# dsmyl6/OpenPyStruct

Measured on AMD Instinct MI355X. Metric: beam FE solves/s (100-elem, batched), higher is better.
Workload: dtype f64

## Files before the change

openpystruct_amd/build.py:

```python
from __future__ import annotations

import os
import shutil
import subprocess
import sys

PKG = os.path.dirname(os.path.abspath(__file__))
ROOT = os.path.dirname(PKG)
CSRC = os.path.join(PKG, "csrc")
LIB = os.path.join(PKG, "lib", "libopenpystruct_amd.so")
SOURCES = [os.path.join(CSRC, "beam_solve.hip"), os.path.join(CSRC, "beam_fat.hip"), os.path.join(CSRC, "sizing_step.hip"),
           os.path.join(CSRC, "beam_residual.hip"), os.path.join(CSRC, "frame_solve.hip"),
           os.path.join(CSRC, "stencil_bn.hip"), os.path.join(CSRC, "flat_adam.hip"),
           os.path.join(CSRC, "fused_loss.hip"), os.path.join(CSRC, "fused_bn.hip"), os.path.join(CSRC, "input_prep.hip"),
           os.path.join(CSRC, "mlp_block.hip"), os.path.join(CSRC, "seq_block.hip"), os.path.join(CSRC, "seq_layer.hip"), os.path.join(CSRC, "mem_bench.hip"), os.path.join(CSRC, "case_draw.hip"),
           os.path.join(CSRC, "bayes_mlp.hip"), os.path.join(CSRC, "beam_vjp.hip"), os.path.join(CSRC, "frame_vjp.hip"), os.path.join(CSRC, "sizing_grad.hip"),
           os.path.join(CSRC, "frame_sizing_grad.hip"), os.path.join(CSRC, "frame_loads.hip"),
           os.path.join(CSRC, "library.hip")]
HEADERS = [os.path.join(CSRC, "lane_common.hpp"), os.path.join(CSRC, "library.hpp"), os.path.join(CSRC, "repack_tiles.hpp"), os.path.join(CSRC, "beam_math.hpp"), os.path.join(CSRC, "beam_adjoint.hpp"), os.path.join(CSRC, "beam_io.hpp"), os.path.join(CSRC, "call_counter.hpp"), os.path.join(CSRC, "dropout_stream.hpp"), os.path.join(CSRC, "input_noise.hpp"), os.path.join(CSRC, "sizing_math.hpp"), os.path.join(CSRC, "frame_wave.hpp"), os.path.join(CSRC, "frame_pack.hpp"), os.path.join(CSRC, "frame_coop.hpp"), os.path.join(CSRC, "frame_adjoint.hpp"), os.path.join(ROOT, "include", "openpystruct_amd.h"),
           os.path.join(ROOT, "include", "openpystruct_amd_frame_vjp.h"), os.path.join(CSRC, "sizing_grad_math.hpp"),
           os.path.join(ROOT, "include", "openpystruct_amd_sizing_grad.h"), os.path.join(CSRC, "frame_sizing_math.hpp"),
           os.path.join(ROOT, "include", "openpystruct_amd_frame_sizing.h"), os.path.join(CSRC, "frame_loads.hpp"),
           os.path.join(ROOT, "include", "openpystruct_amd_frame_loads.h"), os.path.join(CSRC, "frame_stream.hpp")]
ARCH = "gfx950"


def hipcc_path() -> str:
    for cand in (os.environ.get("HIPCC"), shutil.which("hipcc"), "/opt/rocm/bin/hipcc"):
        if cand and os.path.exists(cand):
            return cand
    raise RuntimeError("hipcc not found (set HIPCC or put /opt/rocm/bin on PATH)")


_DEPS_CACHE = {}


def _deps(path: str, seen=None) -> set:
    import re
    seen = set() if seen is None else seen
    path = os.path.normpath(path)
    if path in seen or not os.path.exists(path):
        return seen
    seen.add(path)
    for m in re.finditer(r'^\s*#\s*include\s+"([^"]+)"', open(path).read(), re.M):
        _deps(os.path.join(os.path.dirname(path), m.group(1)), seen)
    return seen


def _flags() -> list:
    return ([f"--offload-arch={ARCH}", "-O3", "-std=c++17", "-fPIC", "-fno-fast-math", "-ffp-contract=off", "-Wall",
             "-Wno-unused-command-line-argument"] + os.environ.get("OPS_AMD_EXTRA_HIPCC_FLAGS", "").split())


def _obj(src: str) -> str:
    return os.path.join(os.path.dirname(LIB), "obj", os.path.splitext(os.path.basename(src))[0] + ".o")


def _stale_objects(force: bool) -> list:
    stamp = os.path.join(os.path.dirname(LIB), "obj", "flags.txt")
    same_flags = os.path.exists(stamp) and open(stamp).read() == " ".join(_flags())
    out = []
    for src in SOURCES:
        o = _obj(src)
        if force or not same_flags or not os.path.exists(o):
            out.append(src)
            continue
        t = os.path.getmtime(o)
        if src not in _DEPS_CACHE:
            _DEPS_CACHE[src] = _deps(src)
        if any(os.path.getmtime(f) > t for f in _DEPS_CACHE[src] | {os.path.abspath(__file__)}):
            out.append(src)
    return out


def needs_build() -> bool:
    if not os.path.exists(LIB) or _stale_objects(False):
        return True
    t = os.path.getmtime(LIB)
    return any(os.path.getmtime(_obj(s)) > t for s in SOURCES)


def build(force: bool = False, verbose: bool = False, jobs: int = 0) -> str:
    if not force and not needs_build():
        return LIB
    from concurrent.futures import ThreadPoolExecutor
    os.makedirs(os.path.join(os.path.dirname(LIB), "obj"), exist_ok=True)
    todo = _stale_objects(force)
    hipcc, flags = hipcc_path(), _flags()
    if verbose:
        flags = ["-Rpass-analysis=kernel-resource-usage"] + flags

    def compile_one(src):
        subprocess.check_call([hipcc] + flags + ["-c", "-o", _obj(src) + ".tmp", src])
        os.replace(_obj(src) + ".tmp", _obj(src))

    jobs = jobs or int(os.environ.get("OPS_AMD_BUILD_JOBS", "0")) or min(len(todo) or 1, max(1, (os.cpu_count() or 2) - 1))
    todo.sort(key=lambda f: -os.path.getsize(f))
    with ThreadPoolExecutor(max_workers=jobs) as ex:
        list(ex.map(compile_one, todo))
    with open(os.path.join(os.path.dirname(LIB), "obj", "flags.txt"), "w") as f:
        f.write(" ".join(_flags()))
    subprocess.check_call([hipcc, f"--offload-arch={ARCH}", "-shared", "-fPIC", "-o", LIB + ".tmp"] + [_obj(s) for s in SOURCES])
    os.replace(LIB + ".tmp", LIB)
    return LIB


if __name__ == "__main__":
    print(build(force="--force" in sys.argv, verbose="-v" in sys.argv))
```

openpystruct_amd/csrc/beam_fat.hip:

```cpp
#include <hip/hip_runtime.h>
#include <stdint.h>

#include <type_traits>

#include "../../include/openpystruct_amd.h"
#include "beam_io.hpp"

namespace opsamd {

template <int PM>
struct FatAcc {
  const double* tab;
  const double* sI;
  const double* sF;
  FixPair bits;
  __device__ __forceinline__ ElemIn elem(int i) const {
    return ElemIn{tab[i], tab[PM + i], tab[2 * PM + i], tab[3 * PM + i], tab[4 * PM + i], tab[5 * PM + i], sI[i], sF[i]};
  }
  __device__ __forceinline__ FixPair fixbits() const { return bits; }
  __device__ __forceinline__ void fence() const { __asm__ volatile("" ::: "memory"); }
};

template <int M, bool FAT>
struct RowOut {
  double* sV; double* sM; double* sv;
  double th[M];
  double vr[FAT ? 1 : M];
  __device__ __forceinline__ void elem(int i, double Vv, double Mv) { sV[i] = Vv; sM[i] = Mv; }
  __device__ __forceinline__ void node(int i, double vv, double tt) {
    if constexpr (FAT) sv[i] = vv; else vr[i] = vv;
    th[i] = tt;
  }
};
template <int M, bool FAT>
struct ParkH {
  double* hx; double* hy;
  Vec2 r[FAT ? 1 : M];
  __device__ __forceinline__ void put(int i, const Vec2& h) {
    if constexpr (FAT) { hx[i] = h.x; hy[i] = h.y; } else r[i] = h;
  }
  __device__ __forceinline__ Vec2 get(int i) const {
    if constexpr (FAT) return Vec2{hx[i], hy[i]}; else return r[i];
  }
};

#ifdef OPS_AMD_TRACE
#define FAT_STAMP(k) stamps[k] = __builtin_amdgcn_s_memrealtime()
#else
#define FAT_STAMP(k) ((void)0)
#endif

struct FatIface {
  const IfacePiece* grp;
  __device__ __forceinline__ IfacePiece piece(int k) const { return grp[k]; }
  __device__ __forceinline__ Mat2 cup(int k) const { return grp[k].cup; }
  __device__ __forceinline__ void fence() const { __asm__ volatile("" ::: "memory"); }
};

template <int P, int M, bool RZ, bool FAT, int PF>
__device__ __forceinline__ void row_solve_lanes(const FatAcc<P * M>& acc, int g, int j, int& bad, RowOut<M, FAT>& out, ParkH<M, FAT>& hs,
                                                IfacePiece* pieces, unsigned lane, unsigned long long* stamps) {
  SegState<M> st;
  std::conditional_t<P == 16 && M == 7, KeepD<M>, KeepNone> keep;
  __asm__ volatile("" ::: "memory");
  seg_condense_pf<M, RZ>(st, acc, bad, keep);
  __asm__ volatile("" ::: "memory");
  FAT_STAMP(6);
  Vec2 uL, uR{0.0, 0.0};
  if constexpr (FAT) {
    pieces[lane] = make_piece<M, RZ>(st, acc.bits);
    __asm__ volatile("" ::: "memory");
    Vec2 u[P];
    iface_thomas<P>(FatIface{pieces + g * P}, u, bad);
    uL = u[0];
#pragma unroll
    for (int k = 1; k < P; ++k) {
      if (j == k) uL = u[k];
      if (j + 1 == k) uR = u[k];
    }
  } else {
    using X = Xch<P>;
    IfaceRow row;
    {
      const Mat2 cup = masked_cup<M, RZ>(st, acc.bits);
      const Sym2 pc = X::template from_minus<1>(st.Scc, (int)lane, j);
      const Vec2 pg = X::template from_minus<1>(st.gc, (int)lane, j);
      const Mat2 pb = X::template from_minus<1>(cup, (int)lane, j);
      row = make_row<M, RZ>(st, cup, pc, pg, pb, acc.bits);
    }
    cr_forward<P, 1>(row, (int)lane, j, bad);
    const Sym2 G = inv_spd(row.D, bad);
    uL = mul(G, row.f);
    if (j != 0) uL = Vec2{0.0, 0.0};
    cr_backward<P, cr_top_level(P)>(row, G, uL, (int)lane, j);
    uR = X::template from_plus<1>(uL, (int)lane, j);
  }
  __asm__ volatile("" ::: "memory");
  FAT_STAMP(7);
  seg_solve_pf<M, RZ, PF>(st, acc, uL, uR, out, hs, keep);
}

struct WordPick {
  bool q1, q2, q3;
  unsigned r;
  __device__ __forceinline__ explicit WordPick(int e0) : q1((e0 >> 5) == 1), q2((e0 >> 5) == 2), q3((e0 >> 5) == 3), r((unsigned)e0 & 31u) {}
};
__device__ __forceinline__ unsigned mask_window(unsigned long long lo, unsigned long long hi, const WordPick& w) {
  const unsigned w0 = (unsigned)lo, w1 = (unsigned)(lo >> 32), w2 = (unsigned)hi, w3 = (unsigned)(hi >> 32);
  unsigned a = w0, b = w1;
  a = w.q1 ? w1 : a;  b = w.q1 ? w2 : b;
  a = w.q2 ? w2 : a;  b = w.q2 ? w3 : b;
  a = w.q3 ? w3 : a;  b = w.q3 ? 0u : b;
  return __builtin_amdgcn_alignbit(b, a, w.r);
}

template <int P, int M, int WPS, bool FAT, bool SIZING>
__device__ __forceinline__ void beam_rows_body(const BeamParams& p, const SizingArgs* sz) {
  constexpr int BPW = 64 / P;
  constexpr int LIVE = BPW * P;
  constexpr int PM = P * M;
  constexpr int NT = (PM + 63) / 64;
  constexpr int ROWS = BPW * PM;
  static_assert(PM <= 128 && PM % 2 == 0 && M + 1 <= 32, "row tiling limits");
  static_assert(FAT || (16 % P == 0 && LIVE == 64), "the lean mapping exchanges over DPP rows");
  constexpr int PF = FAT ? 3 : 1;
#ifdef OPS_AMD_ST
  constexpr int ST = OPS_AMD_ST;
#else
  constexpr int ST = 16;
#endif
  __shared__ double s_tab[6 * PM];
  __shared__ __attribute__((aligned(16))) double s_a[ROWS];
  __shared__ __attribute__((aligned(16))) double s_b[ROWS];
  __shared__ __attribute__((aligned(16))) double s_m[FAT ? ROWS : 2];
  __shared__ __attribute__((aligned(16))) double s_v[FAT ? ROWS : 2];
  __shared__ double s_dummy[M];
  static_assert((6 * PM + (FAT ? 4 : 2) * ROWS + M + 4) * 8 <= 160 * 1024 / (4 * WPS), "LDS per one-wave workgroup");
  static_assert(!FAT || (WPS == 1 && (6 * PM + 4 * ROWS) * 8 > 32 * 1024), "the fat tiling relies on LDS to keep a fifth wave off the CU");

  const unsigned lane = threadIdx.x;
  unsigned long long stamps[8] = {0, 0, 0, 0, 0, 0, 0, 0};
  FAT_STAMP(0);
  const int Ne = p.Ne, N = p.Ne + 1;
  const long beam0 = (long)blockIdx.x * BPW;
  const int nb = (p.B - beam0 < BPW) ? (int)(p.B - beam0) : BPW;
  if (p.active) {
    unsigned any = 0;
    for (int b = 0; b < nb; ++b) any |= p.active[beam0 + b];
    if (!any) return;
  }

  double tx0[NT], tx1[NT];
  const double tE = p.E[0], tw = p.wy[0];
  {
    const __amdgpu_buffer_rsrc_t rx = make_rsrc(p.x, (unsigned)N * 8u);
#pragma unroll
    for (int k = 0; k < NT; ++k) {
      const unsigned e = lane + 64u * k;
      tx0[k] = buf_load_d(rx, e * 8u);
      tx1[k] = buf_load_d(rx, e * 8u + 8u);
    }
  }
  const int g_raw = lane / P, j = lane - g_raw * P, e0 = j * M;
  const bool live = (int)lane < LIVE;
  const int g = live ? g_raw : BPW - 1;
  unsigned char fb0, fb1;
  {
    const __amdgpu_buffer_rsrc_t rf = make_rsrc(p.fix, (unsigned)N);
    fb0 = __builtin_amdgcn_raw_buffer_load_b8(rf, (int)lane, 0, 0);
    fb1 = __builtin_amdgcn_raw_buffer_load_b8(rf, (int)(lane + 64u), 0, 0);
  }
  const int hE = Ne >> 1, hN = N >> 1;
  double2 rI[BPW], rF[BPW];
  double tI = 0.0, tF = 0.0;
  {
    const __amdgpu_buffer_rsrc_t rsF = make_rsrc(p.Fy + beam0 * p.Fy_bs, (unsigned)(((long)(nb - 1) * p.Fy_bs + N) * 8));
    const unsigned oobF = (int)lane < hN ? lane * 16u : 0x40000000u;
    const unsigned tb = lane < (unsigned)nb ? lane : 0u;
    if constexpr (SIZING) {
      const __amdgpu_buffer_rsrc_t rsI = make_rsrc(p.I32 + beam0 * Ne, (unsigned)(nb * Ne) * 4u);
      const unsigned oobI = (int)lane < hE ? lane * 8u : 0x40000000u;
#pragma unroll
      for (int b = 0; b < BPW; ++b) {
        const float2 f = __builtin_bit_cast(float2, __builtin_amdgcn_raw_buffer_load_b64(rsI, (int)((unsigned)(b * Ne) * 4u + oobI), 0, 0));
        rI[b] = make_double2((double)f.x, (double)f.y);
        rF[b] = buf_load_d2(rsF, (unsigned)(b * p.Fy_bs * 8) + oobF);
      }
      if (Ne & 1) tI = (double)__builtin_bit_cast(float, __builtin_amdgcn_raw_buffer_load_b32(rsI, (int)((tb * Ne + Ne - 1) * 4u), 0, 0));
    } else {
      const __amdgpu_buffer_rsrc_t rsI = make_rsrc(p.I + beam0 * p.I_bs, (unsigned)(((long)(nb - 1) * p.I_bs + Ne) * 8));
      const unsigned oobI = (int)lane < hE ? lane * 16u : 0x40000000u;
#pragma unroll
      for (int b = 0; b < BPW; ++b) {
        rI[b] = buf_load_d2(rsI, (unsigned)(b * p.I_bs * 8) + oobI);
        rF[b] = buf_load_d2(rsF, (unsigned)(b * p.Fy_bs * 8) + oobF);
      }
      if (Ne & 1) tI = buf_load_d(rsI, (unsigned)((tb * p.I_bs + Ne - 1) * 8));
    }
    if (N & 1) tF = buf_load_d(rsF, (unsigned)((tb * p.Fy_bs + N - 1) * 8));
  }
  FAT_STAMP(5);
#pragma unroll
  for (int k = 0; k < NT; ++k) {
    const unsigned e = lane + 64u * k;
    if (64 * (k + 1) <= Ne) {
      const double L = tx1[k] - tx0[k];
      const double rl = fast_rcp(L);
      const double c2 = 2.0 * tE * rl, pw = 0.5 * tw * L;
      const double c6 = 3.0 * c2 * rl, c12 = 2.0 * c6 * rl;
      const double mw = pw * L * (1.0 / 6.0);
      s_tab[0 * PM + e] = c2;  s_tab[1 * PM + e] = c6;  s_tab[2 * PM + e] = c12;
      s_tab[3 * PM + e] = rl;  s_tab[4 * PM + e] = pw;  s_tab[5 * PM + e] = mw;
    } else if (e < (unsigned)PM) {
      const bool real = (int)e < Ne, pad = (int)e > Ne;
      const double L = tx1[k] - tx0[k];
      const double rl0 = fast_rcp(real ? L : 1.0);
      const double c2r = 2.0 * tE * rl0, pwr = 0.5 * tw * L;
      const double rl = real ? rl0 : (pad ? 1.0 : 0.0);
      const double c2 = real ? c2r : (pad ? 2.0 : 0.0);
      const double c6 = 3.0 * c2 * rl, c12 = 2.0 * c6 * rl;
      const double pw = real ? pwr : 0.0, mw = pw * L * (1.0 / 6.0);
      s_tab[0 * PM + e] = c2;  s_tab[1 * PM + e] = c6;  s_tab[2 * PM + e] = c12;
      s_tab[3 * PM + e] = rl;  s_tab[4 * PM + e] = pw;  s_tab[5 * PM + e] = mw;
    }
  }
  FixPair bits;
  bool any_rz;
  {
    const unsigned long long v0 = __ballot(fb0 & 1), v1 = __ballot(fb1 & 1);
    const unsigned long long r0 = __ballot(fb0 & 2), r1 = __ballot(fb1 & 2);
    any_rz = (r0 | r1) != 0ull;
    const WordPick pick(e0);
    bits.v = mask_window(v0, v1, pick) & ((2u << M) - 1u);
    bits.t = any_rz ? mask_window(r0, r1, pick) & ((2u << M) - 1u) : 0u;
  }

  if (lane < M) s_dummy[lane] = 0.0;
#pragma unroll
  for (int k = 0; k < (ROWS / 2 + 63) / 64; ++k) {
    const unsigned idx = lane + 64u * k;
    if (k + 1 < (ROWS / 2 + 63) / 64 || idx < ROWS / 2) *reinterpret_cast<double2*>(&s_a[2 * idx]) = make_double2(1.0, 1.0);
  }
#pragma unroll
  for (int b = 0; b < BPW; ++b) {
    if ((int)lane < (b < nb ? hE : 0)) *reinterpret_cast<double2*>(&s_a[b * PM + 2 * lane]) = rI[b];
    if (lane < PM / 2) *reinterpret_cast<double2*>(&s_b[b * PM + 2 * lane]) = rF[b];
  }
  if ((Ne & 1) && (int)lane < nb) s_a[lane * PM + Ne - 1] = tI;
  if ((N & 1) && (int)lane < nb) s_b[lane * PM + N - 1] = tF;
  __syncthreads();
  FAT_STAMP(1);

  FatAcc<PM> acc;
  acc.tab = &s_tab[e0];
  acc.sI = &s_a[g * PM + e0];
  acc.sF = &s_b[g * PM + e0];
  acc.bits = bits;
  int bad = 0;
  RowOut<M, FAT> out;
  out.sV = live ? &s_b[g * PM + e0] : s_dummy;
  out.sM = live ? (FAT ? &s_m[g * PM + e0] : &s_a[g * PM + e0]) : s_dummy;
  out.sv = (FAT && live) ? &s_v[g * PM + e0] : s_dummy;
  ParkH<M, FAT> hs;
  hs.hx = out.sM; hs.hy = out.sv;
  static_assert(!FAT || 64 * sizeof(IfacePiece) <= ROWS * 8, "the interface pieces borrow the moment rows");
  IfacePiece* const pieces = reinterpret_cast<IfacePiece*>(s_m);
  if (any_rz) row_solve_lanes<P, M, true, FAT, PF>(acc, g, j, bad, out, hs, pieces, lane, stamps);
  else        row_solve_lanes<P, M, false, FAT, PF>(acc, g, j, bad, out, hs, pieces, lane, stamps);
  FAT_STAMP(2);

  const unsigned long long bal = __ballot(bad != 0 && live);
  const unsigned long long grp = (P == 64 ? ~0ull : ((1ull << (P % 64)) - 1ull)) << (g * P);
  const bool gbad = (bal & grp) != 0ull;
  if (bal != 0ull && gbad && live) {
    const double qnan = __builtin_nan("");
#pragma unroll
    for (int i = 0; i < M; ++i) {
      out.sV[i] = qnan; out.sM[i] = qnan; out.th[i] = qnan;
      if constexpr (FAT) out.sv[i] = qnan; else out.vr[i] = qnan;
    }
  }
  if (j == 0 && live && g < nb && p.status)
    __hip_atomic_store(&p.status[beam0 + g], gbad ? 1 : 0, __ATOMIC_RELAXED, __HIP_MEMORY_SCOPE_AGENT);
  double* const sth = live ? &s_a[g * PM + e0] : s_dummy;
  if constexpr (FAT) {
#pragma unroll
    for (int i = 0; i < M; ++i) sth[i] = out.th[i];
  }
  wave_lds_fence();
  if constexpr (SIZING) {
    static_assert(!SIZING || !FAT, "the fused epoch uses the lean mapping");
    CaseRegs<2> cr[BPW];
    bool on[BPW];
#pragma unroll
    for (int gb = 0; gb < BPW; ++gb) {
      on[gb] = gb < nb && sz->active[beam0 + gb] != 0;
      if (on[gb]) load_case<2>((int)lane, beam0 + gb, Ne, *sz, cr[gb]);
    }
#pragma unroll
    for (int gb = 0; gb < BPW; ++gb) {
      if (!on[gb]) continue;
      const double* Vb = &s_b[gb * PM];
      const double* Mb = &s_a[gb * PM];
      step_case<2>((int)lane, beam0 + gb, Ne, *sz, cr[gb], [&](int e) { return (float)Vb[e]; }, [&](int e) { return (float)Mb[e]; });
    }
    return;
  }

  const bool two = p.v != nullptr;
  auto read_rows = [&](double2 (&r)[BPW], double& tail, const double* s, int n_) {
    const unsigned lrow = (int)lane < (n_ >> 1) ? lane : 0u;
#pragma unroll
    for (int b = 0; b < BPW; ++b) r[b] = *reinterpret_cast<const double2*>(&s[b * PM + 2 * lrow]);
    tail = s[((int)lane < nb ? lane : 0u) * PM + n_ - 1];
  };
  auto store_rows = [&](auto aux, double* dst, const double2 (&r)[BPW], double tail, int n_) {
    constexpr int AUX = decltype(aux)::value;
    const __amdgpu_buffer_rsrc_t rs = make_rsrc(dst + beam0 * n_, (unsigned)(nb * n_) * 8u);
    const unsigned off = (int)lane < (n_ >> 1) ? lane * 16u : 0x40000000u;
#pragma unroll
    for (int b = 0; b < BPW; ++b)
      buf_store_d2<AUX>(rs, (unsigned)(b * n_) * 8u + off, r[b]);
    if ((n_ & 1) && (int)lane < nb) buf_store_d<AUX>(rs, (unsigned)(lane * n_ + n_ - 1) * 8u, tail);
  };
  auto all_rows = [&](auto aux) {
    double2 ra[BPW], rb[BPW];
    double ta, tb;
    read_rows(ra, ta, s_b, Ne);
    read_rows(rb, tb, FAT ? s_m : s_a, Ne);
    if constexpr (FAT) {
      store_rows(aux, p.V, ra, ta, Ne);
      if (two) read_rows(ra, ta, s_v, N);
      store_rows(aux, p.M, rb, tb, Ne);
      if (two) {
        read_rows(rb, tb, s_a, N);
        store_rows(aux, p.v, ra, ta, N);
        store_rows(aux, p.theta, rb, tb, N);
      }
    } else {
      if (two) {
        wave_lds_fence();
        double* const svv = live ? &s_b[g * PM + e0] : s_dummy;
#pragma unroll
        for (int i = 0; i < M; ++i) { svv[i] = out.vr[i]; sth[i] = out.th[i]; }
      }
      store_rows(aux, p.V, ra, ta, Ne);
      store_rows(aux, p.M, rb, tb, Ne);
      if (two) {
        wave_lds_fence();
        read_rows(ra, ta, s_b, N);
        read_rows(rb, tb, s_a, N);
        store_rows(aux, p.v, ra, ta, N);
        store_rows(aux, p.theta, rb, tb, N);
      }
    }
  };
  if (p.stream_out) all_rows(std::integral_constant<int, 2>{});
  else              all_rows(std::integral_constant<int, ST>{});
#ifdef OPS_AMD_TRACE
  if (p.trace && lane == 0) {
    FAT_STAMP(3);
    stamps[4] = __builtin_amdgcn_s_getreg((4 << 0) | (0 << 6) | ((16 - 1) << 11));
    unsigned long long* q = p.trace + 8 * (unsigned long long)blockIdx.x;
#pragma unroll
    for (int k = 0; k < 8; ++k) q[k] = stamps[k];
  }
#endif
}

template <int P, int M, int WPS, bool FAT>
__global__ __launch_bounds__(64, WPS) void beam_rows_kernel(const BeamParams p) {
  beam_rows_body<P, M, WPS, FAT, false>(p, nullptr);
}
template <int P, int M, int WPS>
__global__ __launch_bounds__(64, WPS) void beam_rows_sizing_kernel(const BeamParams p, const SizingArgs sz) {
  beam_rows_body<P, M, WPS, false, true>(p, &sz);
}

const FatTiling kFatTilings[] = {
    {6, 17, "beam_rows_kernel<6, 17, 1, true>"},
    {16, 7, "beam_rows_kernel<16, 7, 3, false>"},
    {8, 13, "beam_rows_kernel<8, 13, 2, false>"},
};
const int kNumFatTilings = sizeof(kFatTilings) / sizeof(kFatTilings[0]);

hipError_t launch_fat_sizing(const BeamParams& p, const SizingArgs& sz, int P, int M, hipStream_t stream) {
  const unsigned grid = (unsigned)((p.B + 64 / P - 1) / (64 / P));
  if (P == 16 && M == 7) hipLaunchKernelGGL((beam_rows_sizing_kernel<16, 7, 3>), dim3(grid), dim3(64), 0, stream, p, sz);
  else return hipErrorInvalidValue;
  return hipGetLastError();
}

hipError_t launch_fat(const BeamParams& p, int P, int M, hipStream_t stream) {
  const int bpw = 64 / P;
  const unsigned grid = (unsigned)((p.B + bpw - 1) / bpw);
  if (P == 6 && M == 17) hipLaunchKernelGGL((beam_rows_kernel<6, 17, 1, true>), dim3(grid), dim3(64), 0, stream, p);
  else if (P == 16 && M == 7) hipLaunchKernelGGL((beam_rows_kernel<16, 7, 3, false>), dim3(grid), dim3(64), 0, stream, p);
  else if (P == 8 && M == 13) hipLaunchKernelGGL((beam_rows_kernel<8, 13, 2, false>), dim3(grid), dim3(64), 0, stream, p);
  else return hipErrorInvalidValue;
  return hipGetLastError();
}

}
```

openpystruct_amd/csrc/beam_io.hpp:

```cpp
#pragma once
#include <hip/hip_runtime.h>
#include <stdint.h>

#include "beam_math.hpp"
#include "lane_common.hpp"
#include "sizing_math.hpp"

namespace opsamd {

struct BeamParams {
  int B, Ne;
  const double* x;  long x_bs;
  const double* E;  long E_bs;
  const double* I;  long I_bs;
  const uint8_t* fix; long fix_bs;
  const double* Fy; long Fy_bs;
  const double* wy; long wy_bs;
  double* v; double* theta; double* V; double* M;
  int32_t* status;
  const float* I32;
  const uint8_t* active;
  int stream_out;
  int f32_forces;
  int dense;
  unsigned long long* trace;
  unsigned magic_ne, magic_n;
};

struct FatTiling { int P, M; const char* name; };
extern const FatTiling kFatTilings[];
extern const int kNumFatTilings;
hipError_t launch_fat(const BeamParams& p, int P, int M, hipStream_t stream);
hipError_t launch_fat_sizing(const BeamParams& p, const SizingArgs& sz, int P, int M, hipStream_t stream);

template <int SRC>
__device__ __forceinline__ double row_bcast(double x) {
  return __builtin_amdgcn_update_dpp(0.0, x, 0x150 + SRC, 0xF, 0xF, true);
}

template <int P>
struct Xch {
  template <int S>
  static __device__ __forceinline__ double from_minus(double x, int lane, int j) {
    if constexpr (P <= 16 && S < 16) {
      const double r = dpp_mov<0x110 + S>(x);
      if constexpr (P < 16) return j >= S ? r : 0.0;
      return r;
    } else {
      const double r = __shfl(x, lane - S, 64);
      return j >= S ? r : 0.0;
    }
  }
  template <int S>
  static __device__ __forceinline__ double from_plus(double x, int lane, int j) {
    if constexpr (P <= 16 && S < 16) {
      const double r = dpp_mov<0x100 + S>(x);
      if constexpr (P < 16) return j + S < P ? r : 0.0;
      return r;
    } else {
      const double r = __shfl(x, lane + S, 64);
      return j + S < P ? r : 0.0;
    }
  }
  template <int S>
  static __device__ __forceinline__ double top_plus(double x, int lane, int j) {
    if constexpr (P == 16) return row_bcast<S>(x); else return from_plus<S>(x, lane, j);
  }
  template <int S>
  static __device__ __forceinline__ double top_minus(double x, int lane, int j) {
    if constexpr (P == 16) return row_bcast<0>(x); else return from_minus<S>(x, lane, j);
  }
  template <int S> static __device__ __forceinline__ Sym2 from_minus(const Sym2& s, int l, int j) {
    return Sym2{from_minus<S>(s.a, l, j), from_minus<S>(s.b, l, j), from_minus<S>(s.c, l, j)};
  }
  template <int S> static __device__ __forceinline__ Mat2 from_minus(const Mat2& m, int l, int j) {
    return Mat2{from_minus<S>(m.a, l, j), from_minus<S>(m.b, l, j), from_minus<S>(m.c, l, j), from_minus<S>(m.d, l, j)};
  }
  template <int S> static __device__ __forceinline__ Vec2 from_minus(const Vec2& u, int l, int j) {
    return Vec2{from_minus<S>(u.x, l, j), from_minus<S>(u.y, l, j)};
  }
  template <int S> static __device__ __forceinline__ Sym2 from_plus(const Sym2& s, int l, int j) {
    return Sym2{from_plus<S>(s.a, l, j), from_plus<S>(s.b, l, j), from_plus<S>(s.c, l, j)};
  }
  template <int S> static __device__ __forceinline__ Mat2 from_plus(const Mat2& m, int l, int j) {
    return Mat2{from_plus<S>(m.a, l, j), from_plus<S>(m.b, l, j), from_plus<S>(m.c, l, j), from_plus<S>(m.d, l, j)};
  }
  template <int S> static __device__ __forceinline__ Vec2 from_plus(const Vec2& u, int l, int j) {
    return Vec2{from_plus<S>(u.x, l, j), from_plus<S>(u.y, l, j)};
  }
  template <int S> static __device__ __forceinline__ Sym2 top_plus(const Sym2& s, int l, int j) {
    return Sym2{top_plus<S>(s.a, l, j), top_plus<S>(s.b, l, j), top_plus<S>(s.c, l, j)};
  }
  template <int S> static __device__ __forceinline__ Vec2 top_plus(const Vec2& u, int l, int j) {
    return Vec2{top_plus<S>(u.x, l, j), top_plus<S>(u.y, l, j)};
  }
  template <int S> static __device__ __forceinline__ Vec2 top_minus(const Vec2& u, int l, int j) {
    return Vec2{top_minus<S>(u.x, l, j), top_minus<S>(u.y, l, j)};
  }
};

template <int P>
struct XchPerm {
  static __device__ __forceinline__ double fetch(double x, int src_lane) {
    const unsigned long long u = __builtin_bit_cast(unsigned long long, x);
    const int lo = __builtin_amdgcn_ds_bpermute(src_lane << 2, (int)(unsigned)u);
    const int hi = __builtin_amdgcn_ds_bpermute(src_lane << 2, (int)(unsigned)(u >> 32));
    return __builtin_bit_cast(double, ((unsigned long long)(unsigned)hi << 32) | (unsigned)lo);
  }
  template <int S> static __device__ __forceinline__ double from_minus(double x, int lane, int j) { return fetch(x, j >= S ? lane - S : lane); }
// ... 111 lines not shown
```

openpystruct_amd/csrc/beam_solve.hip:

```cpp
#include <hip/hip_runtime.h>
#include <stdint.h>
#include <stdlib.h>

#include <mutex>
#include <type_traits>

#include "../../include/openpystruct_amd.h"
#include "beam_io.hpp"
#include "library.hpp"

namespace opsamd {


struct LdsAcc {
  const double* t2; const double* t6; const double* t12; const double* trl; const double* tpw; const double* tmw;
  const double* sI; const double* sF;
  const double* sZero; int nReal;
  unsigned long long bits;
  __device__ __forceinline__ double c2(int i) const { return t2[i]; }
  __device__ __forceinline__ double c6(int i) const { return t6[i]; }
  __device__ __forceinline__ double c12(int i) const { return t12[i]; }
  __device__ __forceinline__ double rL(int i) const { return trl[i]; }
  __device__ __forceinline__ double pw(int i) const { return tpw[i]; }
  __device__ __forceinline__ double mw(int i) const { return tmw[i]; }
// ... 401 lines not shown
    if (tiling == 0 && !rows && serves && fat_default(f, B, Ne)) return &f;
  }
  return nullptr;
}
static bool is_fat_tiling(int tiling) { return tiling == 6 || (tiling & OPS_AMD_TILING_ROWS) != 0; }

struct OutSeen { const void* p; unsigned long long stamp; };
static std::mutex g_seen_mu;
static OutSeen g_seen[64];
static unsigned g_seen_pos = 0;
static unsigned long long g_traffic = 0;
static bool results_cache_resident(const void* out, unsigned long long call_bytes) {
  constexpr unsigned long long kFits = 224ull << 20;
  std::lock_guard<std::mutex> lock(g_seen_mu);
  bool resident = false, found = false;
  for (OutSeen& e : g_seen) {
    if (e.p == out) {
      resident = (g_traffic - e.stamp) + call_bytes <= kFits;
      e.stamp = g_traffic + call_bytes;
      found = true;
      break;
    }
  }
  if (!found) g_seen[g_seen_pos++ % 64] = OutSeen{out, g_traffic + call_bytes};
  g_traffic += call_bytes;
  return resident;
}

template <int P, int M>
static hipError_t launch(const BeamParams& p, bool shared, hipStream_t stream) {
  constexpr int BPW = 64 / P;
  const unsigned grid = (unsigned)((p.B + BPW - 1) / BPW);
  if (shared && p.dense)
    hipLaunchKernelGGL((beam_solve_kernel<P, M, true, true>), dim3(grid), dim3(64), 0, stream, p);
  else if (shared)
    hipLaunchKernelGGL((beam_solve_kernel<P, M, true, false>), dim3(grid), dim3(64), 0, stream, p);
  else if (p.dense)
    hipLaunchKernelGGL((beam_solve_kernel<P, M, false, true>), dim3(grid), dim3(64), 0, stream, p);
  else
    hipLaunchKernelGGL((beam_solve_kernel<P, M, false, false>), dim3(grid), dim3(64), 0, stream, p);
  return hipGetLastError();
}

template <int P, int M>
static hipError_t launch_sizing(const BeamParams& p, const SizingArgs& sz, bool shared, hipStream_t stream) {
  constexpr int BPW = 64 / P;
  const unsigned grid = (unsigned)((p.B + BPW - 1) / BPW);
  if (shared && p.dense)
    hipLaunchKernelGGL((beam_sizing_epoch_kernel<P, M, true, true>), dim3(grid), dim3(64), 0, stream, p, sz);
  else if (shared)
    hipLaunchKernelGGL((beam_sizing_epoch_kernel<P, M, true, false>), dim3(grid), dim3(64), 0, stream, p, sz);
  else if (p.dense)
    hipLaunchKernelGGL((beam_sizing_epoch_kernel<P, M, false, true>), dim3(grid), dim3(64), 0, stream, p, sz);
  else
    hipLaunchKernelGGL((beam_sizing_epoch_kernel<P, M, false, false>), dim3(grid), dim3(64), 0, stream, p, sz);
  return hipGetLastError();
}

}

using namespace opsamd;

extern "C" {

int ops_amd_max_elements(void) { return 64 * 16 - 1; }

const char* ops_beam_solve_kernel_name(int B, int Ne, int tiling) {
  tiling &= ~OPS_AMD_TILING_STREAM_OUT;
  if (const FatTiling* f = choose_fat(B, Ne, tiling)) return f->name;
  if (is_fat_tiling(tiling)) return "";
  const Tiling* t = choose_tiling(B, Ne, tiling & ~OPS_AMD_TILING_ROWS);
  return t ? t->name_shared : "";
}

static int solve_impl(int B, int Ne, const double* x, long x_bstride, const double* E, long E_bstride,
                      const double* I, long I_bstride, const uint8_t* fix, long fix_bstride,
                      const double* Fy, long Fy_bstride, const double* wy, long wy_bstride, double* v,
                      double* theta, double* V, double* M, int32_t* status, const uint8_t* active, int f32_forces, int tiling,
                      void* stream, const SizingArgs* sz = nullptr) {
  if (B < 0 || Ne < 1) return OPS_AMD_ERR_INVALID_ARG;
  if (B == 0) return OPS_AMD_OK;
  if (!x || !E || (!I && !sz) || !fix || !Fy || !wy || ((!V || !M) && !sz) || ((v == nullptr) != (theta == nullptr))) return OPS_AMD_ERR_INVALID_ARG;
  if (I_bstride < Ne || Fy_bstride < Ne + 1) return OPS_AMD_ERR_INVALID_ARG;
  if ((x_bstride != 0 && x_bstride < Ne + 1) || (fix_bstride != 0 && fix_bstride < Ne + 1) ||
      (E_bstride != 0 && E_bstride < Ne) || (wy_bstride != 0 && wy_bstride < Ne))
    return OPS_AMD_ERR_INVALID_ARG;
  if (Ne > ops_amd_max_elements()) return OPS_AMD_ERR_UNSUPPORTED;
  int stream_out = (tiling & OPS_AMD_TILING_STREAM_OUT) ? 1 : 0;
  tiling &= ~OPS_AMD_TILING_STREAM_OUT;
  if (!sz && !f32_forces) {
    const unsigned long long bytes = (unsigned long long)B * (v ? 4925ull : 3309ull) * (unsigned long long)Ne / 100ull;
    if (!results_cache_resident(V, bytes)) stream_out = 1;
  }
  const bool shared = (x_bstride == 0 && E_bstride == 0 && wy_bstride == 0);
  const uintptr_t align_bits = (uintptr_t)I | (uintptr_t)Fy | (uintptr_t)v | (uintptr_t)theta | (uintptr_t)V | (uintptr_t)M | (sz ? 2 * (uintptr_t)sz->I : 0);
  const bool rows_dense = (I_bstride == Ne) && (Fy_bstride == Ne + 1) && ((align_bits & 15u) == 0);
  const FatTiling* fat = nullptr;
  {
    const bool fat_ok = shared && fix_bstride == 0 && !f32_forces && (sz ? true : !active);
    const FatTiling* f = choose_fat(B, Ne, tiling);
    if (f && fat_ok && (!sz || f->P == 16)) fat = f;
    else if (is_fat_tiling(tiling)) return f ? OPS_AMD_ERR_UNSUPPORTED : OPS_AMD_ERR_INVALID_ARG;
  }
  const Tiling* t = fat ? nullptr : choose_tiling(B, Ne, tiling & ~OPS_AMD_TILING_ROWS);
  if (!t && !fat) return tiling ? OPS_AMD_ERR_INVALID_ARG : OPS_AMD_ERR_UNSUPPORTED;

  BeamParams p{B, Ne, x, x_bstride, E, E_bstride, I, I_bstride, fix, fix_bstride, Fy, Fy_bstride,
               wy, wy_bstride, v, theta, V, M, status, sz ? sz->I : nullptr, active, stream_out, f32_forces, 0, nullptr, 0u, 0u};
#ifdef OPS_AMD_TRACE
  { const char* e = getenv("OPS_AMD_TRACE_PTR"); if (e) p.trace = (unsigned long long*)strtoull(e, nullptr, 0); }
#endif
  {
    const int bpw = 64 / (fat ? fat->P : t->P);
    p.dense = rows_dense && ((bpw * Ne) % 2 == 0) && ((bpw * (Ne + 1)) % 2 == 0);
    p.magic_ne = ((1u << 20) + (unsigned)Ne - 1u) / (unsigned)Ne;
    p.magic_n = ((1u << 20) + (unsigned)Ne) / (unsigned)(Ne + 1);
  }
  hipStream_t s = (hipStream_t)stream;
  hipError_t err = hipSuccess;
  if (fat && sz) err = launch_fat_sizing(p, *sz, fat->P, fat->M, s);
  else if (fat) err = launch_fat(p, fat->P, fat->M, s);
  else if (sz) {
    if (t->P == 8 && t->M == 13) err = launch_sizing<8, 13>(p, *sz, shared, s);
    else if (t->P == 16 && t->M == 7) err = launch_sizing<16, 7>(p, *sz, shared, s);
    else if (t->P == 32 && t->M == 4) err = launch_sizing<32, 4>(p, *sz, shared, s);
    else if (t->P == 64 && t->M == 2) err = launch_sizing<64, 2>(p, *sz, shared, s);
    else if (t->P == 64 && t->M == 4) err = launch_sizing<64, 4>(p, *sz, shared, s);
    else if (t->P == 64 && t->M == 8) err = launch_sizing<64, 8>(p, *sz, shared, s);
    else return OPS_AMD_ERR_UNSUPPORTED;
  }
  else if (t->P == 8 && t->M == 13) err = launch<8, 13>(p, shared, s);
  else if (t->P == 16 && t->M == 7) err = launch<16, 7>(p, shared, s);
  else if (t->P == 32 && t->M == 4) err = launch<32, 4>(p, shared, s);
  else if (t->P == 64 && t->M == 2) err = launch<64, 2>(p, shared, s);
  else if (t->P == 64 && t->M == 4) err = launch<64, 4>(p, shared, s);
  else if (t->P == 64 && t->M == 8) err = launch<64, 8>(p, shared, s);
  else if (t->P == 64 && t->M == 16) err = launch<64, 16>(p, shared, s);
  if (err != hipSuccess) {
    set_last_error(hipGetErrorString(err));
    return OPS_AMD_ERR_LAUNCH;
  }
  return OPS_AMD_OK;
}

int ops_beam_solve_batched_f64(int B, int Ne, const double* x, long x_bstride, const double* E, long E_bstride,
                               const double* I, long I_bstride, const uint8_t* fix, long fix_bstride,
                               const double* Fy, long Fy_bstride, const double* wy, long wy_bstride, double* v,
                               double* theta, double* V, double* M, int32_t* status, int tiling, void* stream) {
  if (B > 0 && Ne >= 1 && (!v || !theta)) return OPS_AMD_ERR_INVALID_ARG;
  return solve_impl(B, Ne, x, x_bstride, E, E_bstride, I, I_bstride, fix, fix_bstride, Fy, Fy_bstride, wy, wy_bstride, v, theta, V, M,
                    status, nullptr, 0, tiling, stream);
}

int ops_beam_solve_forces_f64(int B, int Ne, const double* x, long x_bstride, const double* E, long E_bstride,
                              const double* I, long I_bstride, const uint8_t* fix, long fix_bstride,
                              const double* Fy, long Fy_bstride, const double* wy, long wy_bstride, double* V, double* M,
                              int32_t* status, const uint8_t* active, int tiling, void* stream) {
  return solve_impl(B, Ne, x, x_bstride, E, E_bstride, I, I_bstride, fix, fix_bstride, Fy, Fy_bstride, wy, wy_bstride, nullptr, nullptr,
                    V, M, status, active, 0, tiling, stream);
}

int ops_beam_sizing_epoch_f32(int B, int Ne, const double* x, long x_bstride, const double* E, long E_bstride,
                              const uint8_t* fix, long fix_bstride, const double* Fy, long Fy_bstride, const double* wy,
                              long wy_bstride, float* I, float* I_last, float* exp_avg, float* exp_avg_sq, float* best_loss,
                              int32_t* patience_cnt, int32_t* epochs_run, uint8_t* active, float* last_loss,
                              const ops_sizing_params* hp, const float* schedule, int32_t* status, int tiling, void* stream) {
  if (Ne > 128) return OPS_AMD_ERR_UNSUPPORTED;
  if (!I || !I_last || !exp_avg || !exp_avg_sq || !best_loss || !patience_cnt || !epochs_run || !active || !last_loss || !hp)
    return OPS_AMD_ERR_INVALID_ARG;
  const SizingArgs sz{I, nullptr, I_last, exp_avg, exp_avg_sq, best_loss, patience_cnt, epochs_run, active, last_loss, nullptr, nullptr, *hp, schedule};
  if (tiling == 0 && Ne + 1 <= 16 * 7) {
    const bool rows_ok = x_bstride == 0 && E_bstride == 0 && wy_bstride == 0 && fix_bstride == 0;
    tiling = rows_ok ? (16 | OPS_AMD_TILING_ROWS) : 16;
  }
  return solve_impl(B, Ne, x, x_bstride, E, E_bstride, nullptr, Ne, fix, fix_bstride, Fy, Fy_bstride, wy, wy_bstride, nullptr, nullptr,
                    nullptr, nullptr, status, active, 0, tiling, stream, &sz);
}

int ops_beam_solve_forces_f32(int B, int Ne, const double* x, long x_bstride, const double* E, long E_bstride,
                              const double* I, long I_bstride, const uint8_t* fix, long fix_bstride,
                              const double* Fy, long Fy_bstride, const double* wy, long wy_bstride, float* V32, float* M32,
                              int32_t* status, const uint8_t* active, int tiling, void* stream) {
  return solve_impl(B, Ne, x, x_bstride, E, E_bstride, I, I_bstride, fix, fix_bstride, Fy, Fy_bstride, wy, wy_bstride, nullptr, nullptr,
                    reinterpret_cast<double*>(V32), reinterpret_cast<double*>(M32), status, active, 1, tiling, stream);
// ... 4 lines not shown
```

Before: 895.8 million.

## Pass hot row-kernel args as scalars with kernarg preloading

The row-solve kernels now take the fields they touch first (Ne, B, I, Fy, strides, x, E, wy) as separate scalar kernel arguments, and beam_fat.hip is compiled with an LLVM flag that preloads the first 14 kernarg dwords into SGPRs. The rarely used pointers move into a tail struct. The fix-bit loads are moved after the I/Fy loads, and strides are narrowed to 32-bit, with new host checks that reject oversized strides. The aim is to cut kernarg load latency at wave start for this short, launch-bound kernel. The cost is extra build-system plumbing for per-file flags and a narrower range of accepted strides.

```diff
diff --git a/openpystruct_amd/build.py b/openpystruct_amd/build.py
--- a/openpystruct_amd/build.py
+++ b/openpystruct_amd/build.py
@@ -23,6 +23,7 @@
            os.path.join(ROOT, "include", "openpystruct_amd_frame_sizing.h"), os.path.join(CSRC, "frame_loads.hpp"),
            os.path.join(ROOT, "include", "openpystruct_amd_frame_loads.h"), os.path.join(CSRC, "frame_stream.hpp")]
 ARCH = "gfx950"
+FILE_FLAGS = {"beam_fat.hip": ["-mllvm", "-amdgpu-kernarg-preload-count=14"]}
 
 
 def hipcc_path() -> str:
@@ -47,9 +48,17 @@
     return seen
 
 
+def _file_flags(src: str) -> list:
+    return FILE_FLAGS.get(os.path.basename(src), [])
+
+
 def _flags() -> list:
     return ([f"--offload-arch={ARCH}", "-O3", "-std=c++17", "-fPIC", "-fno-fast-math", "-ffp-contract=off", "-Wall",
              "-Wno-unused-command-line-argument"] + os.environ.get("OPS_AMD_EXTRA_HIPCC_FLAGS", "").split())
+
+
+def _flags_stamp() -> str:
+    return " ".join(_flags()) + "".join(f"\n{k}: {' '.join(v)}" for k, v in sorted(FILE_FLAGS.items()))
 
 
 def _obj(src: str) -> str:
@@ -58,7 +67,7 @@
 
 def _stale_objects(force: bool) -> list:
     stamp = os.path.join(os.path.dirname(LIB), "obj", "flags.txt")
-    same_flags = os.path.exists(stamp) and open(stamp).read() == " ".join(_flags())
+    same_flags = os.path.exists(stamp) and open(stamp).read() == _flags_stamp()
     out = []
     for src in SOURCES:
         o = _obj(src)
@@ -91,7 +100,7 @@
         flags = ["-Rpass-analysis=kernel-resource-usage"] + flags
 
     def compile_one(src):
-        subprocess.check_call([hipcc] + flags + ["-c", "-o", _obj(src) + ".tmp", src])
+        subprocess.check_call([hipcc] + flags + _file_flags(src) + ["-c", "-o", _obj(src) + ".tmp", src])
         os.replace(_obj(src) + ".tmp", _obj(src))
 
     jobs = jobs or int(os.environ.get("OPS_AMD_BUILD_JOBS", "0")) or min(len(todo) or 1, max(1, (os.cpu_count() or 2) - 1))
@@ -99,7 +108,7 @@
     with ThreadPoolExecutor(max_workers=jobs) as ex:
         list(ex.map(compile_one, todo))
     with open(os.path.join(os.path.dirname(LIB), "obj", "flags.txt"), "w") as f:
-        f.write(" ".join(_flags()))
+        f.write(_flags_stamp())
     subprocess.check_call([hipcc, f"--offload-arch={ARCH}", "-shared", "-fPIC", "-o", LIB + ".tmp"] + [_obj(s) for s in SOURCES])
     os.replace(LIB + ".tmp", LIB)
     return LIB
diff --git a/openpystruct_amd/csrc/beam_fat.hip b/openpystruct_amd/csrc/beam_fat.hip
--- a/openpystruct_amd/csrc/beam_fat.hip
+++ b/openpystruct_amd/csrc/beam_fat.hip
@@ -45,7 +45,7 @@
 };
 
 #ifdef OPS_AMD_TRACE
-#define FAT_STAMP(k) stamps[k] = __builtin_amdgcn_s_memrealtime()
+#define FAT_STAMP(k) (__builtin_amdgcn_sched_barrier(0), stamps[k] = __builtin_amdgcn_s_memrealtime(), __builtin_amdgcn_sched_barrier(0))
 #else
 #define FAT_STAMP(k) ((void)0)
 #endif
@@ -115,7 +115,7 @@
 }
 
 template <int P, int M, int WPS, bool FAT, bool SIZING>
-__device__ __forceinline__ void beam_rows_body(const BeamParams& p, const SizingArgs* sz) {
+__device__ __forceinline__ void beam_rows_body(const RowsHead& p, const RowsTail& t, const SizingArgs* sz) {
   constexpr int BPW = 64 / P;
   constexpr int LIVE = BPW * P;
   constexpr int PM = P * M;
@@ -142,16 +142,17 @@
   unsigned long long stamps[8] = {0, 0, 0, 0, 0, 0, 0, 0};
   FAT_STAMP(0);
   const int Ne = p.Ne, N = p.Ne + 1;
+  const long I_bs = p.I_bs, Fy_bs = p.Fy_bs;
   const long beam0 = (long)blockIdx.x * BPW;
   const int nb = (p.B - beam0 < BPW) ? (int)(p.B - beam0) : BPW;
-  if (p.active) {
+  if (SIZING && t.active) {
     unsigned any = 0;
-    for (int b = 0; b < nb; ++b) any |= p.active[beam0 + b];
+    for (int b = 0; b < nb; ++b) any |= t.active[beam0 + b];
     if (!any) return;
   }
-
+  const double tE = p.E[0], tw = p.wy[0];
+  __builtin_amdgcn_sched_barrier(0);
   double tx0[NT], tx1[NT];
-  const double tE = p.E[0], tw = p.wy[0];
   {
     const __amdgpu_buffer_rsrc_t rx = make_rsrc(p.x, (unsigned)N * 8u);
 #pragma unroll
@@ -164,42 +165,42 @@
   const int g_raw = lane / P, j = lane - g_raw * P, e0 = j * M;
   const bool live = (int)lane < LIVE;
   const int g = live ? g_raw : BPW - 1;
-  unsigned char fb0, fb1;
-  {
-    const __amdgpu_buffer_rsrc_t rf = make_rsrc(p.fix, (unsigned)N);
-    fb0 = __builtin_amdgcn_raw_buffer_load_b8(rf, (int)lane, 0, 0);
-    fb1 = __builtin_amdgcn_raw_buffer_load_b8(rf, (int)(lane + 64u), 0, 0);
-  }
   const int hE = Ne >> 1, hN = N >> 1;
   double2 rI[BPW], rF[BPW];
   double tI = 0.0, tF = 0.0;
   {
-    const __amdgpu_buffer_rsrc_t rsF = make_rsrc(p.Fy + beam0 * p.Fy_bs, (unsigned)(((long)(nb - 1) * p.Fy_bs + N) * 8));
+    const __amdgpu_buffer_rsrc_t rsF = make_rsrc(p.Fy + beam0 * Fy_bs, (unsigned)(((long)(nb - 1) * Fy_bs + N) * 8));
     const unsigned oobF = (int)lane < hN ? lane * 16u : 0x40000000u;
     const unsigned tb = lane < (unsigned)nb ? lane : 0u;
     if constexpr (SIZING) {
-      const __amdgpu_buffer_rsrc_t rsI = make_rsrc(p.I32 + beam0 * Ne, (unsigned)(nb * Ne) * 4u);
+      const __amdgpu_buffer_rsrc_t rsI = make_rsrc(static_cast<const float*>(p.I) + beam0 * Ne, (unsigned)(nb * Ne) * 4u);
       const unsigned oobI = (int)lane < hE ? lane * 8u : 0x40000000u;
 #pragma unroll
       for (int b = 0; b < BPW; ++b) {
         const float2 f = __builtin_bit_cast(float2, __builtin_amdgcn_raw_buffer_load_b64(rsI, (int)((unsigned)(b * Ne) * 4u + oobI), 0, 0));
         rI[b] = make_double2((double)f.x, (double)f.y);
-        rF[b] = buf_load_d2(rsF, (unsigned)(b * p.Fy_bs * 8) + oobF);
+        rF[b] = buf_load_d2(rsF, (unsigned)(b * Fy_bs * 8) + oobF);
       }
       if (Ne & 1) tI = (double)__builtin_bit_cast(float, __builtin_amdgcn_raw_buffer_load_b32(rsI, (int)((tb * Ne + Ne - 1) * 4u), 0, 0));
     } else {
-      const __amdgpu_buffer_rsrc_t rsI = make_rsrc(p.I + beam0 * p.I_bs, (unsigned)(((long)(nb - 1) * p.I_bs + Ne) * 8));
+      const __amdgpu_buffer_rsrc_t rsI = make_rsrc(static_cast<const double*>(p.I) + beam0 * I_bs, (unsigned)(((long)(nb - 1) * I_bs + Ne) * 8));
       const unsigned oobI = (int)lane < hE ? lane * 16u : 0x40000000u;
 #pragma unroll
       for (int b = 0; b < BPW; ++b) {
-        rI[b] = buf_load_d2(rsI, (unsigned)(b * p.I_bs * 8) + oobI);
-        rF[b] = buf_load_d2(rsF, (unsigned)(b * p.Fy_bs * 8) + oobF);
+        rI[b] = buf_load_d2(rsI, (unsigned)(b * I_bs * 8) + oobI);
+        rF[b] = buf_load_d2(rsF, (unsigned)(b * Fy_bs * 8) + oobF);
       }
-      if (Ne & 1) tI = buf_load_d(rsI, (unsigned)((tb * p.I_bs + Ne - 1) * 8));
-    }
-    if (N & 1) tF = buf_load_d(rsF, (unsigned)((tb * p.Fy_bs + N - 1) * 8));
+      if (Ne & 1) tI = buf_load_d(rsI, (unsigned)((tb * I_bs + Ne - 1) * 8));
+    }
+    if (N & 1) tF = buf_load_d(rsF, (unsigned)((tb * Fy_bs + N - 1) * 8));
   }
   FAT_STAMP(5);
+  unsigned char fb0, fb1;
+  {
+    const __amdgpu_buffer_rsrc_t rf = make_rsrc(t.fix, (unsigned)N);
+    fb0 = __builtin_amdgcn_raw_buffer_load_b8(rf, (int)lane, 0, 0);
+    fb1 = __builtin_amdgcn_raw_buffer_load_b8(rf, (int)(lane + 64u), 0, 0);
+  }
 #pragma unroll
   for (int k = 0; k < NT; ++k) {
     const unsigned e = lane + 64u * k;
@@ -280,8 +281,8 @@
       if constexpr (FAT) out.sv[i] = qnan; else out.vr[i] = qnan;
     }
   }
-  if (j == 0 && live && g < nb && p.status)
-    __hip_atomic_store(&p.status[beam0 + g], gbad ? 1 : 0, __ATOMIC_RELAXED, __HIP_MEMORY_SCOPE_AGENT);
+  if (j == 0 && live && g < nb && t.status)
+    __hip_atomic_store(&t.status[beam0 + g], gbad ? 1 : 0, __ATOMIC_RELAXED, __HIP_MEMORY_SCOPE_AGENT);
   double* const sth = live ? &s_a[g * PM + e0] : s_dummy;
   if constexpr (FAT) {
 #pragma unroll
@@ -307,7 +308,7 @@
     return;
   }
 
-  const bool two = p.v != nullptr;
+  const bool two = t.v != nullptr;
   auto read_rows = [&](double2 (&r)[BPW], double& tail, const double* s, int n_) {
     const unsigned lrow = (int)lane < (n_ >> 1) ? lane : 0u;
 #pragma unroll
@@ -329,13 +330,13 @@
     read_rows(ra, ta, s_b, Ne);
     read_rows(rb, tb, FAT ? s_m : s_a, Ne);
     if constexpr (FAT) {
-      store_rows(aux, p.V, ra, ta, Ne);
+      store_rows(aux, t.V, ra, ta, Ne);
       if (two) read_rows(ra, ta, s_v, N);
-      store_rows(aux, p.M, rb, tb, Ne);
+      store_rows(aux, t.M, rb, tb, Ne);
       if (two) {
         read_rows(rb, tb, s_a, N);
-        store_rows(aux, p.v, ra, ta, N);
-        store_rows(aux, p.theta, rb, tb, N);
+        store_rows(aux, t.v, ra, ta, N);
+        store_rows(aux, t.theta, rb, tb, N);
       }
     } else {
       if (two) {
@@ -344,24 +345,24 @@
 #pragma unroll
         for (int i = 0; i < M; ++i) { svv[i] = out.vr[i]; sth[i] = out.th[i]; }
       }
-      store_rows(aux, p.V, ra, ta, Ne);
-      store_rows(aux, p.M, rb, tb, Ne);
+      store_rows(aux, t.V, ra, ta, Ne);
+      store_rows(aux, t.M, rb, tb, Ne);
       if (two) {
         wave_lds_fence();
         read_rows(ra, ta, s_b, N);
         read_rows(rb, tb, s_a, N);
-        store_rows(aux, p.v, ra, ta, N);
-        store_rows(aux, p.theta, rb, tb, N);
+        store_rows(aux, t.v, ra, ta, N);
+        store_rows(aux, t.theta, rb, tb, N);
       }
     }
   };
-  if (p.stream_out) all_rows(std::integral_constant<int, 2>{});
+  if (t.stream_out) all_rows(std::integral_constant<int, 2>{});
   else              all_rows(std::integral_constant<int, ST>{});
 #ifdef OPS_AMD_TRACE
-  if (p.trace && lane == 0) {
+  if (t.trace && lane == 0) {
     FAT_STAMP(3);
     stamps[4] = __builtin_amdgcn_s_getreg((4 << 0) | (0 << 6) | ((16 - 1) << 11));
-    unsigned long long* q = p.trace + 8 * (unsigned long long)blockIdx.x;
+    unsigned long long* q = t.trace + 8 * (unsigned long long)blockIdx.x;
 #pragma unroll
     for (int k = 0; k < 8; ++k) q[k] = stamps[k];
   }
@@ -369,12 +370,13 @@
 }
 
 template <int P, int M, int WPS, bool FAT>
-__global__ __launch_bounds__(64, WPS) void beam_rows_kernel(const BeamParams p) {
-  beam_rows_body<P, M, WPS, FAT, false>(p, nullptr);
+__global__ __launch_bounds__(64, WPS) void beam_rows_kernel(int Ne, int B, const void* I, const double* Fy, unsigned I_bs, unsigned Fy_bs,
+                                                           const double* x, const double* E, const double* wy, const RowsTail t) {
+  beam_rows_body<P, M, WPS, FAT, false>(RowsHead{Ne, B, I, Fy, I_bs, Fy_bs, x, E, wy}, t, nullptr);
 }
 template <int P, int M, int WPS>
-__global__ __launch_bounds__(64, WPS) void beam_rows_sizing_kernel(const BeamParams p, const SizingArgs sz) {
-  beam_rows_body<P, M, WPS, false, true>(p, &sz);
+__global__ __launch_bounds__(64, WPS) void beam_rows_sizing_kernel(const RowsHead h, const RowsTail t, const SizingArgs sz) {
+  beam_rows_body<P, M, WPS, false, true>(h, t, &sz);
 }
 
 const FatTiling kFatTilings[] = {
@@ -384,9 +386,17 @@
 };
 const int kNumFatTilings = sizeof(kFatTilings) / sizeof(kFatTilings[0]);
 
+static RowsHead rows_head(const BeamParams& p, const void* I) { return RowsHead{p.Ne, p.B, I, p.Fy, (unsigned)p.I_bs, (unsigned)p.Fy_bs, p.x, p.E, p.wy}; }
+static RowsTail rows_tail(const BeamParams& p) { return RowsTail{p.fix, p.v, p.theta, p.V, p.M, p.status, p.active, p.stream_out, p.trace}; }
+static void launch_rows(void (*kernel)(int, int, const void*, const double*, unsigned, unsigned, const double*, const double*, const double*, RowsTail),
+                        unsigned grid, hipStream_t stream, const BeamParams& p) {
+  const RowsHead h = rows_head(p, p.I);
+  hipLaunchKernelGGL(kernel, dim3(grid), dim3(64), 0, stream, h.Ne, h.B, h.I, h.Fy, h.I_bs, h.Fy_bs, h.x, h.E, h.wy, rows_tail(p));
+}
+
 hipError_t launch_fat_sizing(const BeamParams& p, const SizingArgs& sz, int P, int M, hipStream_t stream) {
   const unsigned grid = (unsigned)((p.B + 64 / P - 1) / (64 / P));
-  if (P == 16 && M == 7) hipLaunchKernelGGL((beam_rows_sizing_kernel<16, 7, 3>), dim3(grid), dim3(64), 0, stream, p, sz);
+  if (P == 16 && M == 7) hipLaunchKernelGGL((beam_rows_sizing_kernel<16, 7, 3>), dim3(grid), dim3(64), 0, stream, rows_head(p, p.I32), rows_tail(p), sz);
   else return hipErrorInvalidValue;
   return hipGetLastError();
 }
@@ -394,9 +404,9 @@
 hipError_t launch_fat(const BeamParams& p, int P, int M, hipStream_t stream) {
   const int bpw = 64 / P;
   const unsigned grid = (unsigned)((p.B + bpw - 1) / bpw);
-  if (P == 6 && M == 17) hipLaunchKernelGGL((beam_rows_kernel<6, 17, 1, true>), dim3(grid), dim3(64), 0, stream, p);
-  else if (P == 16 && M == 7) hipLaunchKernelGGL((beam_rows_kernel<16, 7, 3, false>), dim3(grid), dim3(64), 0, stream, p);
-  else if (P == 8 && M == 13) hipLaunchKernelGGL((beam_rows_kernel<8, 13, 2, false>), dim3(grid), dim3(64), 0, stream, p);
+  if (P == 6 && M == 17) launch_rows(beam_rows_kernel<6, 17, 1, true>, grid, stream, p);
+  else if (P == 16 && M == 7) launch_rows(beam_rows_kernel<16, 7, 3, false>, grid, stream, p);
+  else if (P == 8 && M == 13) launch_rows(beam_rows_kernel<8, 13, 2, false>, grid, stream, p);
   else return hipErrorInvalidValue;
   return hipGetLastError();
 }
diff --git a/openpystruct_amd/csrc/beam_io.hpp b/openpystruct_amd/csrc/beam_io.hpp
--- a/openpystruct_amd/csrc/beam_io.hpp
+++ b/openpystruct_amd/csrc/beam_io.hpp
@@ -25,6 +25,22 @@
   int dense;
   unsigned long long* trace;
   unsigned magic_ne, magic_n;
+};
+
+struct RowsHead {
+  int Ne, B;
+  const void* I;
+  const double* Fy;
+  unsigned I_bs, Fy_bs;
+  const double* x; const double* E; const double* wy;
+};
+struct RowsTail {
+  const uint8_t* fix;
+  double* v; double* theta; double* V; double* M;
+  int32_t* status;
+  const uint8_t* active;
+  int stream_out;
+  unsigned long long* trace;
 };
 
 struct FatTiling { int P, M; const char* name; };
diff --git a/openpystruct_amd/csrc/beam_solve.hip b/openpystruct_amd/csrc/beam_solve.hip
--- a/openpystruct_amd/csrc/beam_solve.hip
+++ b/openpystruct_amd/csrc/beam_solve.hip
@@ -507,6 +507,7 @@
   if (B == 0) return OPS_AMD_OK;
   if (!x || !E || (!I && !sz) || !fix || !Fy || !wy || ((!V || !M) && !sz) || ((v == nullptr) != (theta == nullptr))) return OPS_AMD_ERR_INVALID_ARG;
   if (I_bstride < Ne || Fy_bstride < Ne + 1) return OPS_AMD_ERR_INVALID_ARG;
+  if (I_bstride >= (1l << 31) || Fy_bstride >= (1l << 31)) return OPS_AMD_ERR_INVALID_ARG;
   if ((x_bstride != 0 && x_bstride < Ne + 1) || (fix_bstride != 0 && fix_bstride < Ne + 1) ||
       (E_bstride != 0 && E_bstride < Ne) || (wy_bstride != 0 && wy_bstride < Ne))
     return OPS_AMD_ERR_INVALID_ARG;
@@ -524,7 +525,8 @@
   {
     const bool fat_ok = shared && fix_bstride == 0 && !f32_forces && (sz ? true : !active);
     const FatTiling* f = choose_fat(B, Ne, tiling);
-    if (f && fat_ok && (!sz || f->P == 16)) fat = f;
+    const bool rows_fit = f && (unsigned long long)(64 / f->P - 1) * (unsigned long long)(I_bstride > Fy_bstride ? I_bstride : Fy_bstride) + Ne + 1 < (1ull << 29);
+    if (f && fat_ok && rows_fit && (!sz || f->P == 16)) fat = f;
     else if (is_fat_tiling(tiling)) return f ? OPS_AMD_ERR_UNSUPPORTED : OPS_AMD_ERR_INVALID_ARG;
   }
   const Tiling* t = fat ? nullptr : choose_tiling(B, Ne, tiling & ~OPS_AMD_TILING_ROWS);
```

New measurement: 963.1 million, median of 6. 7.5% higher.
